# mcahny/vps

Hardware: AMD Instinct MI355X
Metric: frames/sec FuseTrack 1024x2048 (higher is better)
Workload: dtype f32-grade: f16x3 split operands (fp16 pair with scaled residual, 22 significand bits) on MFMA, f32 accumulate

## Files before the change

### include/vps_hip.h

```cpp
#ifndef VPS_HIP_H
#define VPS_HIP_H

#include <stdint.h>

#ifdef __cplusplus
extern "C" {
#endif

int vps_abi_version(void);
const char* vps_build_info(void);

enum { VPS_ACT_NONE = 0, VPS_ACT_RELU = 1, VPS_ACT_LEAKY = 2 };
enum { VPS_PREC_F32 = 0, VPS_PREC_BF16 = 1, VPS_PREC_BF16X3 = 2, VPS_PREC_BF16X6 = 3, VPS_PREC_F16X3 = 4 };

typedef struct vps_conv_desc {
    const float* in;
    int32_t N, H, W;
    int32_t in_ld;
    int32_t in_coff;
    int32_t cin_pad;
    const float* w;
    int32_t cout, cout_pad, kpad;
    int32_t KH, KW, stride;
    int32_t pad_y[2], pad_x[2];
// ... 6 lines not shown
    const float* scale;
    const float* shift;
    const float* res;
    int32_t res_ld, res_coff, res_shift;
    int32_t act;
    float slope;
    const float* offset;
    int32_t off_ld;
    int32_t tile_n;
    int32_t ksplit;
    float* ws;
    int32_t prec;
    const void* w_split;
    int32_t korder;
    int32_t* status;
    double* gn_stats;
    int32_t gn_cpg, gn_rep;
    int32_t* tile_counter;
    const void* w_thin;
} vps_conv_desc;

int vps_conv2d(const vps_conv_desc* d, void* stream);

typedef struct vps_tensor4 {
    float* p;
    int64_t sn, sc, sh, sw;
} vps_tensor4;

int vps_resample2d(vps_tensor4 in, vps_tensor4 flow, vps_tensor4 out,
                   int B, int C, int H, int W, void* stream);

int vps_channelnorm(vps_tensor4 in, vps_tensor4 out, int B, int C, int H, int W, void* stream);

int vps_correlation(const float* in1, int ld1, int coff1, const float* in2, int ld2, int coff2,
                    float* out, int out_ld, int out_coff,
                    int N, int H, int W, int C, int max_disp, int stride2,
                    int act, float slope, void* stream);
int vps_correlation_f16(const float* in1, int ld1, int coff1, const float* in2, int ld2, int coff2,
                        float* out, int out_ld, int out_coff, int N, int H, int W, int C,
                        int max_disp, int stride2, int act, float slope, int32_t* status, void* stream);

int vps_flow_warp(const float* in, int in_ld, int in_coff, const float* flow, int flow_ld, int flow_coff,
                  float* out, int out_ld, int out_coff, int N, int H, int W, int C, void* stream);

int vps_nchw_to_nhwc(const float* in, float* out, int out_ld, int out_coff, int N, int C, int H, int W,
                     int Cpad, void* stream);
// ... 189 lines not shown
```

### vps_amd/csrc/conv_mfma.hip

```cpp
#include "conv_common.h"

namespace {
template <int TM, int TN, int WAVES_M, int WAVES_N, bool DEFORM>
__global__ __launch_bounds__(256, 2)
void conv_mfma_f32_kernel(const vps_conv_desc d, const int M, const int tiles_m, const int tiles_n,
                          const int ksteps_per_split) {
    constexpr int BN = WAVES_N * TN * 32;
    static_assert(WAVES_M * TM * 32 == BM, "block M tile must be 128");
    static_assert(WAVES_M * WAVES_N == 4, "4 wavefronts per block");
    constexpr int NB = BN / 32;

    __shared__ __attribute__((aligned(16))) float As[BM * LDS_LD];
    __shared__ __attribute__((aligned(16))) float Bs[BN * LDS_LD];

    const int t = threadIdx.x;
    int swz = xcd_swizzle(blockIdx.x, gridDim.x);
    int tile_n, tile_m, cls, split;
    decode_tile(d, swz, tiles_n, tiles_m, tile_n, tile_m, cls, split);

    const int py = cls / d.os_x, px = cls - py * d.os_x;
    const int pad_y = d.pad_y[py], pad_x = d.pad_x[px];
    const float* __restrict__ wcls = d.w + (size_t)cls * d.cout_pad * d.kpad;

    const int H = d.H, W = d.W, KH = d.KH, KW = d.KW, cin_pad = d.cin_pad;
// ... 711 lines not shown
        });
        return;
    }
#define VPS_CONV_LAUNCH(KERNEL) hipLaunchKernelGGL((KERNEL), grid, block, 0, s, d, p.M, p.tiles_m, p.tiles_n, p.per_split)
    if (p.kernel == CONV_K_F32) {
        if (d.offset) VPS_CONV_LAUNCH((conv_mfma_f32_kernel<TM, TN, WAVES_M, WAVES_N, true>));
        else VPS_CONV_LAUNCH((conv_mfma_f32_kernel<TM, TN, WAVES_M, WAVES_N, false>));
        return;
    }
    const bool tapmajor = d.korder == 0 && d.KH * d.KW > 1;
    with_prec<true>(d.prec, [&](auto mode) {
        constexpr int MODE = decltype(mode)::value;
        if (d.offset) VPS_CONV_LAUNCH((conv_mfma_bf16p_kernel<TM, TN, WAVES_M, WAVES_N, MODE, false, true>));
        else if (tapmajor) VPS_CONV_LAUNCH((conv_mfma_bf16p_kernel<TM, TN, WAVES_M, WAVES_N, MODE, true>));
        else VPS_CONV_LAUNCH((conv_mfma_bf16p_kernel<TM, TN, WAVES_M, WAVES_N, MODE, false>));
    });
#undef VPS_CONV_LAUNCH
}

conv_switches conv_switches_now(const vps_conv_desc& d) {
    const auto on = [](const char* name) { const char* const e = getenv(name); return !(e && atoi(e) == 0); };
    const auto not0 = [](const char* name) { const char* const e = getenv(name); return !(e && e[0] == '0'); };
    static const bool s2_halo = not0("VPS_S2_HALO"), thin = on("VPS_THIN"), debug_occ = getenv("VPS_DEBUG_OCC") != nullptr;
    conv_switches sw = {true, true, true, true, s2_halo, thin, debug_occ};
    if (d.prec != VPS_PREC_F16X3) return sw;
    if (d.tile_n == 32) {
        if (d.cout > 16) sw.n32 = not0("VPS_N32");
        else if (d.nclass == 4) sw.n16t = on("VPS_N16T");
    } else if (d.tile_n <= 128 && d.KH == 1) sw.pw = on("VPS_PW");
    else if (d.tile_n == 128 && d.KH == 3 && d.stride == 1) sw.h8p = on("VPS_H8P");
    return sw;
}

const conv_limits& conv_limits_once(const bool debug) {
    static const conv_limits lim = [debug] {
        conv_limits l = {};
        int dev = 0;
        (void)hipGetDevice(&dev);
        (void)hipDeviceGetAttribute(&l.cus, hipDeviceAttributeMultiprocessorCount, dev);
        vpsi_conv_pw_limits(l, debug);
        vpsi_conv_thin_limits(l, debug);
        if (debug) vpsi_conv_q_debug_occ();
        return l;
    }();
    return lim;
}

}

extern "C" int vps_conv2d(const vps_conv_desc* dp, void* stream) {
    if (!dp) return VPS_EARG(1);
    const vps_conv_desc& d = *dp;
    if (const int e = vpsi_conv_check(d)) return e;
    const conv_switches sw = conv_switches_now(d);
    const conv_plan p = vpsi_conv_plan(d, conv_limits_once(sw.debug_occ), sw);
    hipStream_t s = (hipStream_t)stream;
    switch (p.kernel) {
        case CONV_K_NONE: return p.err;
        case CONV_K_SMALL3X3V: case CONV_K_SMALL_BATCHED: case CONV_K_SMALL: vpsi_launch_conv_small(d, p, s); break;
        case CONV_K_THIN: vpsi_launch_conv_thin(d, p, s); break;
        case CONV_K_DCN256:
            hipLaunchKernelGGL((conv_mfma_bf16p_kernel<2, 4, 2, 2, VPS_PREC_F16X3, false, true>), dim3(p.grid), dim3(p.block), 0, s, d, p.M, p.tiles_m, p.tiles_n, p.per_split);
            break;
        case CONV_K_N16T: case CONV_K_N32: case CONV_K_N16: vpsi_launch_conv_n16(d, p, s); break;
        case CONV_K_H8S2: vpsi_launch_conv_h8s2(d, p, s); break;
        case CONV_K_H8P: vpsi_launch_conv_h8p(d, p, s); break;
        case CONV_K_H8: vpsi_launch_conv_h8(d, p, s); break;
        case CONV_K_PW: vpsi_launch_conv_pw(d, p, s); break;
        case CONV_K_Q: vpsi_launch_conv_q(d, p, s); break;
        default:
// ... 12 lines not shown
```

### vps_amd/csrc/conv_plan.cpp

```cpp
#include "conv_plan.h"
#include <stdint.h>

namespace {

constexpr int BM = 128, BK = 32;

inline int cdiv(long a, long b) { return (int)((a + b - 1) / b); }
inline size_t in_bytes(const vps_conv_desc& d) { return (size_t)d.N * d.H * d.W * d.in_ld * sizeof(float); }
inline size_t out_bytes(const vps_conv_desc& d) { return (size_t)d.N * d.Ho * d.Wo * d.out_ld * sizeof(float); }
inline bool two_plane(int prec) { return prec == VPS_PREC_F16X3 || prec == VPS_PREC_BF16X3 || prec == VPS_PREC_BF16; }

constexpr int H8_MIN_CHUNKS = 3;
constexpr int PW_MIN_ROUNDS = 2;

conv_plan fail(conv_plan p, int n) { p.kernel = CONV_K_NONE; p.err = VPS_EARG(n); return p; }

conv_plan plan_small(const vps_conv_desc& d, conv_plan p) {
    p.block = 256;
    p.G = 1; p.logG = 0;
    while (p.G < 64 && p.G < (d.cin_pad >> 2)) { p.G <<= 1; ++p.logG; }
    const size_t wbytes = (size_t)(d.cout <= 2 ? 2 : 4) * d.kpad * sizeof(float);
    if (d.KH == 3 && d.KW == 3 && d.stride == 1 && d.nclass == 1 && d.pad_y[0] == 1 && d.pad_x[0] == 1 && d.Ho == d.H && d.Wo == d.W &&
        wbytes <= 150 * 1024 && (d.cout <= 2 || d.cout_pad >= 4) && in_bytes(d) < 0xFFFFFFF0ull &&
        (long)d.N * d.H * d.W < 0x7fffffffL) {
// ... 35 lines not shown
    while (i < 4 && !(d.KH == conv_thin_shapes[i].ks && d.stride == conv_thin_shapes[i].s && d.cin_pad == conv_thin_shapes[i].c4)) ++i;
    if (i == 4) return false;
    const int ph = conv_thin_shapes[i].ph;
    const int tiles_x = (d.Qw + 31) / 32, tiles_y = (d.Qh + ph - 1) / ph;
    const long ntiles = (long)d.N * tiles_x * tiles_y;
    if (ntiles < 512 || ntiles > 0x7fffffffL) return false;
    const int resident = (lim.thin_per_cu[i] > 0 ? lim.thin_per_cu[i] : 1) * (lim.cus > 0 ? lim.cus : 256);
    const long rounds = (ntiles + resident - 1) / resident;
    p.kernel = CONV_K_THIN; p.thin = i; p.tiles_n = tiles_x; p.tiles_m = tiles_y; p.ntiles = (int)ntiles;
    p.grid = (unsigned)((ntiles + rounds - 1) / rounds); p.block = 256;
    return true;
}

bool plan_pw(const vps_conv_desc& d, const conv_limits& lim, const conv_switches& sw, conv_plan& p) {
    if (!sw.pw || d.prec != VPS_PREC_F16X3 || d.offset || d.KH != 1 || d.KW != 1 || d.nclass != 1 || d.ksplit != 1 || d.gn_stats) return false;
    if (d.pad_y[0] || d.pad_x[0] || (d.cin_pad & 31) || d.kpad != d.cin_pad || (d.tile_n != 128 && d.tile_n != 64)) return false;
    const int nk = d.kpad / BK;
    if (nk < 2 || (nk & 1)) return false;
    if (d.Ho != d.Qh || d.Wo != d.Qw || (d.stride == 1 && (d.H != d.Qh || d.W != d.Qw))) return false;
    if (((d.cout | d.out_ld | d.out_coff) & 3) || ((uintptr_t)d.out & 15) || out_bytes(d) >= 0xFFFFFE00ull) return false;
    if (d.res && (((d.res_ld | d.res_coff) & 3) || ((uintptr_t)d.res & 15) || d.res_shift < 0 || d.res_shift > 4 ||
                  (size_t)d.N * (d.Ho >> d.res_shift) * (d.Wo >> d.res_shift) * d.res_ld * sizeof(float) >= 0xFFFFFE00ull)) return false;
    if (in_bytes(d) >= 0xFFFFFE00ull) return false;
    const int per_cu = lim.pw_per_cu[d.tile_n == 128 ? 1 : 0];
    const int resident = (per_cu > 0 ? per_cu : 1) * (lim.cus > 0 ? lim.cus : 256);
    const long total = (long)p.tiles_m * p.tiles_n;
    const int unit = 8 * p.tiles_n;
    if (resident < unit || total < (long)PW_MIN_ROUNDS * resident) return false;
    const long rounds = (total + resident - 1) / resident;
    long grid = (total + rounds - 1) / rounds;
    grid = (grid + unit - 1) / unit * unit;
    if (grid > resident) grid = resident / unit * unit;
    const int mper = (int)(grid / unit);
    p.kernel = CONV_K_PW; p.grid = (unsigned)grid; p.nk = nk; p.nit = (p.tiles_m + mper * 8 - 1) / (mper * 8);
    return true;
}

}

const conv_thin_shape conv_thin_shapes[4] = {{8, 3, 1, 8}, {12, 3, 1, 8}, {4, 7, 2, 8}, {12, 7, 2, 4}};

const char* vpsi_conv_kernel_name(int kernel) {
    static const char* const names[] = {"none", "small3x3v", "small_batched", "small", "thin", "dcn256", "n16t", "n32", "n16",
                                        "h8s2", "h8p", "h8", "halo", "pw", "q", "f32", "bf16p"};
    return kernel >= 0 && kernel <= CONV_K_BF16P ? names[kernel] : "?";
}

int vpsi_conv_check(const vps_conv_desc& d) {
    if (!d.in || !d.out) return VPS_EARG(2);
    if (d.prec < VPS_PREC_F32 || d.prec > VPS_PREC_F16X3) return VPS_EARG(12);
    if (d.prec == VPS_PREC_F32 ? !d.w : !d.w_split) return VPS_EARG(13);
    if ((d.in_ld & 3) || (d.in_coff & 3) || (d.cin_pad & 3) || d.cin_pad <= 0) return VPS_EARG(3);
    if ((d.kpad % BK) || d.kpad < d.KH * d.KW * d.cin_pad || (d.korder != 0 && d.korder != 1)) return VPS_EARG(4);
    if (d.korder == 1 && d.kpad != d.KH * d.KW * ((d.cin_pad + BK - 1) / BK) * BK) return VPS_EARG(14);
    if (d.tile_n != 32 && d.tile_n != 64 && d.tile_n != 128 && !(d.tile_n == 256 && d.offset && d.prec == VPS_PREC_F16X3 && d.korder == 1)) return VPS_EARG(5);
    if (d.cout_pad % d.tile_n || d.cout > d.cout_pad || d.cout <= 0) return VPS_EARG(6);
    if (d.nclass != d.os_y * d.os_x || d.nclass < 1 || d.os_y > 2 || d.os_x > 2) return VPS_EARG(7);
// ... 56 lines not shown
                           d.pad_x[0] >= 0 && d.pad_x[0] <= 1 && d.pad_x[1] >= 0 && d.pad_x[1] <= 1;
        p.tiles_m = (int)tiles2d8; p.block = 512;
        if (fused && d.cout <= 16) { p.kernel = CONV_K_N16T; p.grid = (unsigned)tiles2d8; }
        else { p.kernel = d.cout > 16 ? CONV_K_N32 : CONV_K_N16; p.grid = (unsigned)(tiles2d8 * d.nclass); }
    } else if (h8s2) {
        p.kernel = CONV_K_H8S2; p.tiles_m = (int)tiles2d8; p.block = 512; p.grid = (unsigned)(tiles2d8 * tiles_n * d.ksplit);
    } else if (h8) {
        p.kernel = sw.h8p && d.prec == VPS_PREC_F16X3 && d.KH == 3 ? CONV_K_H8P : CONV_K_H8;
        p.tiles_m = (int)tiles2d8; p.block = 512; p.grid = (unsigned)(tiles2d8 * tiles_n * d.nclass * d.ksplit);
    } else if (halo) {
        const long nblk2 = tiles2d * tiles_n * d.nclass * d.ksplit;
        if (nblk2 > 0x7fffffffL) return fail(p, 21);
        p.kernel = CONV_K_HALO; p.tiles_m = (int)tiles2d; p.grid = (unsigned)nblk2;
    } else {
        p.grid = (unsigned)nblk;
        const bool tapmajor = d.korder == 0 && ntap > 1;
        const bool q_ok = BN >= 64 && !tapmajor;
        if (q_ok && plan_pw(d, lim, sw, p)) return p;
        if (q_ok && !d.offset && two_plane(d.prec)) p.kernel = CONV_K_Q;
        else p.kernel = d.prec == VPS_PREC_F32 ? CONV_K_F32 : CONV_K_BF16P;
    }
    return p;
}
```

### vps_amd/csrc/conv_plan.h

```cpp
#pragma once
#include <stddef.h>
#include "../../include/vps_hip.h"

#ifndef VPS_EARG
#define VPS_EARG(x) (-1000 - (x))
#endif

enum conv_kernel {
    CONV_K_NONE = 0,
    CONV_K_SMALL3X3V,
    CONV_K_SMALL_BATCHED,
    CONV_K_SMALL,
    CONV_K_THIN,
    CONV_K_DCN256,
    CONV_K_N16T,
    CONV_K_N32,
    CONV_K_N16,
    CONV_K_H8S2,
    CONV_K_H8P,
    CONV_K_H8,
    CONV_K_HALO,
    CONV_K_PW,
    CONV_K_Q,
    CONV_K_F32,
    CONV_K_BF16P,
};

struct conv_plan {
    int kernel;
    int err;
    int M;
    int tiles_m, tiles_n;
    int per_split;
    int chunks_per_split;
    unsigned grid, block;
    size_t smem;
    int nk, nit;
    int G, logG, nslot;
    int runs_per_row, total_runs;
    int thin;
    int ntiles;
    bool needs_reduce;
    bool reduce_v4;
};

struct conv_limits {
    int cus;
    int pw_per_cu[2];
    int thin_per_cu[4];
};

struct conv_switches {
    bool pw;
    bool h8p;
    bool n16t;
    bool n32;
    bool s2_halo;
    bool thin;
    bool debug_occ;
};

struct conv_thin_shape { int c4, ks, s, ph; };
extern const conv_thin_shape conv_thin_shapes[4];

int vpsi_conv_check(const vps_conv_desc& d);
conv_plan vpsi_conv_plan(const vps_conv_desc& d, const conv_limits& lim, const conv_switches& sw);
const char* vpsi_conv_kernel_name(int kernel);

#ifdef __HIPCC__
void vpsi_launch_conv_small(const vps_conv_desc& d, const conv_plan& p, hipStream_t s);
void vpsi_launch_conv_thin(const vps_conv_desc& d, const conv_plan& p, hipStream_t s);
void vpsi_launch_conv_n16(const vps_conv_desc& d, const conv_plan& p, hipStream_t s);
void vpsi_launch_conv_h8(const vps_conv_desc& d, const conv_plan& p, hipStream_t s);
void vpsi_launch_conv_h8p(const vps_conv_desc& d, const conv_plan& p, hipStream_t s);
void vpsi_launch_conv_h8s2(const vps_conv_desc& d, const conv_plan& p, hipStream_t s);
void vpsi_launch_conv_pw(const vps_conv_desc& d, const conv_plan& p, hipStream_t s);
void vpsi_launch_conv_q(const vps_conv_desc& d, const conv_plan& p, hipStream_t s);
void vpsi_conv_pw_limits(conv_limits& lim, bool debug);
void vpsi_conv_thin_limits(conv_limits& lim, bool debug);
void vpsi_conv_q_debug_occ();
#endif
```

### vps_amd/csrc/conv_pw.hip

```cpp
#include "conv_common.h"
#include <cstdio>

namespace {

constexpr int PMODE = VPS_PREC_F16X3;

template <int TN, bool HAS_RES, int NKU>
__global__ __launch_bounds__(256, 2)
void conv_pw_kernel(const vps_conv_desc d, const int M, const int tiles_m, const int tiles_n, const int nk, const int nit) {
    constexpr int TM = 2, WAVES_N = 2;
    constexpr int BN = WAVES_N * TN * 32;
    typedef Split<PMODE> SM;
    typedef _Float16 elem_t;
    typedef vec8<elem_t> x8;
    typedef vec4<elem_t> x4;
    constexpr int NSA = SM::NSA, NSB = SM::NSB, NLB = SM::NLB, NT = SM::NT;
    static_assert(NSA == 2 && NLB == 2 && NSB == 3 && NT == 3, "f16x3");
    constexpr int ABUF = NSA * BM * LDS_LDH;
    constexpr int NFRAG = NLB * 2 * (BN / 32);
    constexpr int BBUF = NFRAG * 512;
    static_assert((NFRAG * 64) % 256 == 0, "whole 16-byte chunks per thread");
    constexpr int NBL = NFRAG * 64 / 256;
    constexpr int NST = TM * TN * 4;

    __shared__ __attribute__((aligned(16))) elem_t As[2 * ABUF];
    __shared__ __attribute__((aligned(16))) elem_t Bs[2 * BBUF];
    __shared__ __attribute__((aligned(16))) float scsh[2 * BN];

    const int t = threadIdx.x;
    const int lane = t & 63;
    const int wave = __builtin_amdgcn_readfirstlane(t >> 6);
    const int wm = wave / WAVES_N, wn = wave - wm * WAVES_N;

    const int G = gridDim.x;
    const int xcd = blockIdx.x & 7, bj = blockIdx.x >> 3;
    const int tile_n = bj % tiles_n, mlocal = bj / tiles_n, mper = (G >> 3) / tiles_n;

    const int k4 = t & 7;
    const int r0 = t >> 3;
    const int nbt = d.cout_pad >> 5, kst = d.kpad >> 4;
    const size_t wplane = (size_t)nbt * kst * 512;
    const __amdgpu_buffer_rsrc_t wrsrc = make_rsrc(d.w_split, (unsigned)(wplane * NSB * sizeof(elem_t)));
    const unsigned wbase = (unsigned)((((size_t)(tile_n * (BN / 32)) * kst) * 512) * sizeof(elem_t));
    const unsigned wlane = (unsigned)lane * 16u;
    const __amdgpu_buffer_rsrc_t arsrc = make_rsrc(d.in, (unsigned)((size_t)d.N * d.H * d.W * d.in_ld * sizeof(float)));
    const __amdgpu_buffer_rsrc_t orsrc = make_rsrc(d.out, (unsigned)((size_t)d.N * d.Ho * d.Wo * d.out_ld * sizeof(float)));
    const int rs = d.res_shift;
    const __amdgpu_buffer_rsrc_t rrsrc = make_rsrc(HAS_RES ? d.res : d.in, HAS_RES ? (unsigned)((size_t)d.N * (d.Ho >> rs) * (d.Wo >> rs) * d.res_ld * sizeof(float)) : 0u);
    const unsigned ld4 = (unsigned)d.in_ld * 4u;
    const unsigned acoff = (unsigned)(d.in_coff + k4 * 4) * 4u;
    const bool plain = d.stride == 1;

    int lk = 0, lit = 0, bk = 0;
    unsigned rowoff[4];
    auto set_rows = [&](const int it) {
        const int tm = (it * mper + mlocal) * 8 + xcd;
#pragma unroll
        for (int i = 0; i < 4; ++i) {
            const int m = tm * BM + r0 + 32 * i;
            const bool ok = tm < tiles_m && m < M;
            unsigned pix = (unsigned)m;
            if (!plain) {
                const int mm = ok ? m : 0;
                const int qx = mm % d.Qw, tq = mm / d.Qw;
                const int qy = tq % d.Qh, n = tq / d.Qh;
                pix = (unsigned)((n * d.H + qy * d.stride) * d.W + qx * d.stride);
            }
            rowoff[i] = ok ? pix * ld4 + acoff : 0xFFFFFFF0u;
        }
    };
    f32x4 areg[2][4];
    x8 breg[2][NBL];
    float amax = 0.f;

    auto load_A = [&](const int slot) {
        const unsigned koff = (unsigned)lk * (BK * 4u);
#pragma unroll
        for (int i = 0; i < 4; ++i)
            areg[slot][i] = buffer_load16<f32x4>(arsrc, rowoff[i] != 0xFFFFFFF0u ? rowoff[i] + koff : 0xFFFFFFF0u, 0u);
        if (++lk == nk) {
            lk = 0;
            ++lit;
            set_rows(lit);
        }
    };
    auto load_B = [&](const int slot) {
#pragma unroll
        for (int j = 0; j < NBL; ++j) {
            const int f = wave + 4 * j, bcol = f % (BN / 32), pm = f / (BN / 32);
            breg[slot][j] = buffer_load16<x8>(wrsrc, wlane, wbase + (unsigned)(((size_t)(pm >> 1) * wplane + ((size_t)bcol * kst + 2 * bk + (pm & 1)) * 512) * sizeof(elem_t)));
        }
        if (++bk == nk) bk = 0;
    };
    auto store_A = [&](const int i, const int buf, const int slot) {
        x4 sp[NSA];
        split_act<PMODE>(areg[slot][i], sp, amax);
        const int row = r0 + 32 * i;
#pragma unroll
        for (int p = 0; p < NSA; ++p)
            *reinterpret_cast<x4*>(&As[buf * ABUF + p * (BM * LDS_LDH) + row * LDS_LDH + (((k4 >> 1) ^ lds_swz(row)) << 3) + ((k4 & 1) << 2)]) = sp[p];
    };
    auto store_B = [&](const int j, const int buf, const int slot) {
        *reinterpret_cast<x8*>(&Bs[buf * BBUF + (t + 256 * j) * 8]) = breg[slot][j];
    };

    const int frag_row = (wm * TM * 32 + (lane & 31)) * LDS_LDH;
    const int frag_sw = lds_swz(lane & 31);
    const int frag_chunk[2] = {(((lane >> 5)) ^ frag_sw) << 3, ((2 + (lane >> 5)) ^ frag_sw) << 3};
    x8 af[2][NSA][TM];
    x8 bf[NSB][TN];
    auto read_A = [&](const int m, const int buf) {
#pragma unroll
        for (int p = 0; p < NSA; ++p)
#pragma unroll
            for (int a = 0; a < TM; ++a)
                af[m][p][a] = *reinterpret_cast<const x8*>(&As[buf * ABUF + p * (BM * LDS_LDH) + a * 32 * LDS_LDH + frag_row + frag_chunk[m]]);
    };
    auto read_B = [&](const int m, const int p, const int buf) {
#pragma unroll
        for (int b = 0; b < TN; ++b)
            bf[p][b] = *reinterpret_cast<const x8*>(&Bs[buf * BBUF + (((p * 2 + m) * (BN / 32)) + wn * TN + b) * 512 + lane * 8]);
    };

    f32x16 acc[TM][TN];

    {
        const int c = t & (BN - 1);
        const int co = tile_n * BN + c;
        float v = t < BN ? 1.f : 0.f;
        if (co < d.cout) {
            if (t < BN && d.scale) v = d.scale[co];
            if (t >= BN && d.shift) v = d.shift[co];
        }
        if (t < 2 * BN) scsh[t] = v;
    }
    set_rows(0);
    load_B(0);
    load_A(0);
#pragma unroll
    for (int i = 0; i < 4; ++i) store_A(i, 0, 0);
#pragma unroll
    for (int j = 0; j < NBL; ++j) store_B(j, 0, 0);
    load_B(1);
    load_A(1);
    if constexpr (NKU == 2) {
#pragma unroll
        for (int j = 0; j < NBL; ++j) store_B(j, 1, 1);
    } else {
        load_B(0);
    }
    load_A(0);
    {
        const u32x4 z = {0u, 0u, 0u, 0u};
#pragma unroll
        for (int i = 0; i < NST; ++i) __builtin_amdgcn_raw_buffer_store_b128(z, orsrc, (int)(0xFFFFFE00u + 16u * (unsigned)i), 0, 0);
    }
    __syncthreads();

    constexpr int NM1 = NT * TM * TN;
    constexpr int NW = 8;

    auto kstep = [&](auto cur_tag, auto first_tag) {
        constexpr int cur = decltype(cur_tag)::value;
        constexpr bool first = decltype(first_tag)::value;
        constexpr int slot = cur ^ 1;
        read_A(0, cur);
#pragma unroll
        for (int p = 0; p < NLB; ++p) read_B(0, p, cur);
        read_A(1, cur);
        __builtin_amdgcn_sched_barrier(0);
        auto prep = [&](const int q) {
            if (SM::PB[q] >= NLB) {
#pragma unroll
                for (int b = 0; b < TN; ++b) bf[SM::PB[q]][b] = derive_weight_plane<PMODE>(bf[0][b]);
            }
        };
#pragma unroll
        for (int q = 0; q < NT; ++q) {
            prep(q);
#pragma unroll
            for (int a = 0; a < TM; ++a)
#pragma unroll
                for (int b = 0; b < TN; ++b) {
                    if (first && q == 0) {
                        const f32x16 z = {0.f, 0.f, 0.f, 0.f, 0.f, 0.f, 0.f, 0.f, 0.f, 0.f, 0.f, 0.f, 0.f, 0.f, 0.f, 0.f};
                        acc[a][b] = split_mfma<PMODE>(bf[SM::PB[q]][b], af[0][SM::PA[q]][a], z);
                    } else {
                        acc[a][b] = split_mfma<PMODE>(bf[SM::PB[q]][b], af[0][SM::PA[q]][a], acc[a][b]);
                    }
                }
            bool last_use = SM::PB[q] < NLB;
#pragma unroll
            for (int q2 = q + 1; q2 < NT; ++q2) last_use = last_use && SM::PB[q2] != SM::PB[q];
#pragma unroll
            for (int q2 = q + 1; q2 < NT; ++q2) last_use = last_use && !(SM::PB[q] == 0 && SM::PB[q2] >= NLB);
            if (last_use) {
                __builtin_amdgcn_sched_barrier(0);
                read_B(1, SM::PB[q], cur);
                __builtin_amdgcn_sched_barrier(0);
            }
        }
        auto work = [&](const int w) {
            if (w < 4) store_A(w, cur ^ 1, slot);
            else if (w == 4) {
                if constexpr (NKU != 2) {
#pragma unroll
                    for (int j = 0; j < (NBL + 1) / 2; ++j) store_B(j, cur ^ 1, slot);
                }
            } else if (w == 5) {
                if constexpr (NKU != 2) {
#pragma unroll
                    for (int j = (NBL + 1) / 2; j < NBL; ++j) store_B(j, cur ^ 1, slot);
                }
            } else if (w == 6) {
                if constexpr (NKU != 2) load_B(slot);
            } else load_A(slot);
        };
        int mf = 0;
#pragma unroll
        for (int q = 0; q < NT; ++q) {
            prep(q);
#pragma unroll
            for (int a = 0; a < TM; ++a)
#pragma unroll
                for (int b = 0; b < TN; ++b) {
                    acc[a][b] = split_mfma<PMODE>(bf[SM::PB[q]][b], af[1][SM::PA[q]][a], acc[a][b]);
                    ++mf;
#pragma unroll
                    for (int w = 0; w < NW; ++w) {
                        const int pos = ((w + 1) * NM1 + NW) / (NW + 1);
                        if (mf == (pos < 1 ? 1 : (pos > NM1 ? NM1 : pos))) {
                            __builtin_amdgcn_sched_barrier(0);
                            work(w);
                            __builtin_amdgcn_sched_barrier(0);
                        }
                    }
                }
        }
        __syncthreads();
    };

    const int prow = lane & 31;
    const int cl = wn * TN * 32 + 4 * (lane >> 5);
    const unsigned ocol4 = (unsigned)(d.out_coff + tile_n * BN + cl) * 4u;
    const unsigned rcol4 = (unsigned)(d.res_coff + tile_n * BN + cl) * 4u;
    const float ns = d.act == VPS_ACT_RELU ? 0.f : (d.act == VPS_ACT_LEAKY ? d.slope : 1.f);
    auto epilogue = [&](const int it) {
        const int tm = (it * mper + mlocal) * 8 + xcd;
        unsigned ooff[TM], roff[TM];
#pragma unroll
        for (int a = 0; a < TM; ++a) {
            const int m = tm * BM + wm * TM * 32 + a * 32 + prow;
            const bool inside = tm < tiles_m && m < M;
            ooff[a] = inside ? (unsigned)m * ((unsigned)d.out_ld * 4u) + ocol4 : 0xFFFFFFF0u;
            roff[a] = 0xFFFFFFF0u;
            if constexpr (HAS_RES) {
                unsigned rp = (unsigned)m;
                if (rs) {
                    const int mm = inside ? m : 0;
                    const int qx = mm % d.Qw, tq = mm / d.Qw;
                    const int qy = tq % d.Qh, n = tq / d.Qh;
                    rp = (unsigned)((n * (d.Ho >> rs) + (qy >> rs)) * (d.Wo >> rs) + (qx >> rs));
                }
                roff[a] = inside ? rp * ((unsigned)d.res_ld * 4u) + rcol4 : 0xFFFFFFF0u;
            }
        }
        f32x4 rv[HAS_RES ? TM : 1][HAS_RES ? TN : 1][4];
        if constexpr (HAS_RES) {
#pragma unroll
            for (int a = 0; a < TM; ++a)
#pragma unroll
                for (int b = 0; b < TN; ++b)
#pragma unroll
                    for (int g = 0; g < 4; ++g) {
                        const bool cok = tile_n * BN + cl + b * 32 + 8 * g < d.cout;
// ... 50 lines not shown
            kstep(C0{}, FF{});
            kstep(C1{}, FF{});
            ks += 2;
            if (ks == nk) {
                epilogue(it);
                ++it;
                ks = 0;
#pragma unroll
                for (int a = 0; a < TM; ++a)
#pragma unroll
                    for (int b = 0; b < TN; ++b)
#pragma unroll
                        for (int r = 0; r < 16; ++r) acc[a][b][r] = 0.f;
            }
        }
    }
    report_range<PMODE>(d, amax);
}

}

__attribute__((visibility("hidden")))
void vpsi_conv_pw_limits(conv_limits& lim, bool debug) {
    (void)hipOccupancyMaxActiveBlocksPerMultiprocessor(&lim.pw_per_cu[0], conv_pw_kernel<1, false, 0>, 256, 0);
    (void)hipOccupancyMaxActiveBlocksPerMultiprocessor(&lim.pw_per_cu[1], conv_pw_kernel<2, false, 0>, 256, 0);
    if (debug) for (int tn = 1; tn <= 2; ++tn) fprintf(stderr, "[vps] pointwise kernel <TN %d>: %d blocks/CU\n", tn, lim.pw_per_cu[tn - 1]);
}

__attribute__((visibility("hidden")))
void vpsi_launch_conv_pw(const vps_conv_desc& d, const conv_plan& p, hipStream_t s) {
    const int tn = d.tile_n == 128 ? 2 : 1;
#define VPS_PW_LAUNCH(TNV, RESV, NKV) hipLaunchKernelGGL((conv_pw_kernel<TNV, RESV, NKV>), dim3(p.grid), dim3(p.block), 0, s, d, p.M, p.tiles_m, p.tiles_n, p.nk, p.nit)
#define VPS_PW_NK(TNV, RESV)                                         \
    do {                                                             \
        if (p.nk == 2) VPS_PW_LAUNCH(TNV, RESV, 2);                  \
        else if (p.nk == 4) VPS_PW_LAUNCH(TNV, RESV, 4);             \
        else if (p.nk == 8) VPS_PW_LAUNCH(TNV, RESV, 8);             \
        else VPS_PW_LAUNCH(TNV, RESV, 0);                            \
    } while (0)
    if (d.res) { if (tn == 2) VPS_PW_NK(2, true); else VPS_PW_NK(1, true); }
    else { if (tn == 2) VPS_PW_NK(2, false); else VPS_PW_NK(1, false); }
#undef VPS_PW_NK
#undef VPS_PW_LAUNCH
}
```

### vps_amd/hip.py

```python
import ctypes
import os
from ctypes import (POINTER, Structure, byref, c_char_p, c_double, c_float, c_int, c_int32, c_int64, c_uint64,
                    c_void_p)

import torch

_HERE = os.path.dirname(os.path.abspath(__file__))
LIB_PATH = os.environ.get('VPS_HIP_LIB') or os.path.join(_HERE, 'csrc', 'libvpship.so')
ABI_VERSION = 21

ACT_NONE, ACT_RELU, ACT_LEAKY = 0, 1, 2
PREC_F32, PREC_BF16, PREC_BF16X3, PREC_BF16X6, PREC_F16X3 = 0, 1, 2, 3, 4

SYMBOLS = [
    'vps_abi_version', 'vps_build_info', 'vps_conv2d', 'vps_resample2d', 'vps_channelnorm', 'vps_correlation',
    'vps_flow_warp', 'vps_nchw_to_nhwc', 'vps_nhwc_to_nchw', 'vps_resize', 'vps_pool3x3s2', 'vps_bfp_gather',
    'vps_bfp_scatter', 'vps_bfp_scatter_all', 'vps_axpb', 'vps_flow_prep', 'vps_flow_prep_pad', 'vps_flow_stage', 'vps_flow_stage_full', 'vps_groupnorm_relu', 'vps_groupnorm_apply', 'vps_tcea_temporal',
    'vps_tcea_modulate', 'vps_tcea_modulate_ld', 'vps_correlation_f16', 'vps_roi_align', 'vps_nms_batched', 'vps_delta2bbox', 'vps_bbox_overlaps',
    'vps_row_softmax', 'vps_mask_count', 'vps_mask_commit', 'vps_mask_removal', 'vps_mask_removal_dep', 'vps_mask_removal_hist', 'vps_frame_tail', 'vps_mask_level', 'vps_panoptic_combine',
    'vps_panoptic_combine_dev', 'vps_rpn_select', 'vps_rpn_collect', 'vps_maskroi_select', 'vps_maskroi_finish', 'vps_track_assign', 'vps_pan_instances',
    'vps_unify_hist', 'vps_unify_tables', 'vps_unify_write', 'vps_image_prep', 'vps_resize_u8', 'vps_segment_stats', 'vps_segment_paint', 'vps_pair_count',
    'vps_png_info', 'vps_png_decode_bgr8', 'vps_jpeg_info', 'vps_jpeg_decode_coef', 'vps_jpeg_reconstruct',
    'vps_png_encode_bound', 'vps_png_deflate',
    'vps_png_inflate', 'vps_png_reconstruct_ws', 'vps_png_reconstruct', 'vps_png_reconstruct_block_rows',
    'vps_unify_tables_image', 'vps_segment_stats_ch', 'vps_segment_paint_ch', 'vps_sseg_confusion',
    'vps_overlay_render', 'vps_jpeg_quant_tables', 'vps_jpeg_encode_bound', 'vps_jpeg_encode_coef', 'vps_jpeg_write_bound', 'vps_jpeg_write',
    'vps_flow_max_radius', 'vps_flow_colour',
    'vps_rle_runs', 'vps_rle_runs_ws', 'vps_rle_band_rows', 'vps_rle_strings', 'vps_rle_strings_bound',
]


class ConvDesc(Structure):
    _fields_ = [
        ('inp', c_void_p), ('N', c_int32), ('H', c_int32), ('W', c_int32),
        ('in_ld', c_int32), ('in_coff', c_int32), ('cin_pad', c_int32),
        ('w', c_void_p), ('cout', c_int32), ('cout_pad', c_int32), ('kpad', c_int32),
        ('KH', c_int32), ('KW', c_int32), ('stride', c_int32),
        ('pad_y', c_int32 * 2), ('pad_x', c_int32 * 2),
# ... 46 lines not shown
def load_host():
    load()
    return _host


def load():
    global _lib
    if _lib is not None:
        return _lib
    if not os.path.exists(LIB_PATH):
        raise VpsHipError('libvpship.so not found at %s — build it with `python -c "import __graft_entry__ as g; '
                          'g.build()"` or `make -C vps_amd/csrc`. There is no CPU fallback.' % LIB_PATH)
    lib = ctypes.PyDLL(LIB_PATH)
    missing = [s for s in SYMBOLS if not hasattr(lib, s)]
    if missing:
        raise VpsHipError('libvpship.so is missing symbols: %s' % missing)
    lib.vps_abi_version.restype = c_int
    lib.vps_build_info.restype = c_char_p
    if lib.vps_abi_version() != ABI_VERSION:
        raise VpsHipError('libvpship.so ABI %d != binding ABI %d' % (lib.vps_abi_version(), ABI_VERSION))
    for s in SYMBOLS[2:]:
        getattr(lib, s).restype = c_int
    lib.vps_conv2d.argtypes = [POINTER(ConvDesc), c_void_p]
    lib.vps_resample2d.argtypes = [Tensor4, Tensor4, Tensor4, c_int, c_int, c_int, c_int, c_void_p]
    lib.vps_channelnorm.argtypes = [Tensor4, Tensor4, c_int, c_int, c_int, c_int, c_void_p]
    lib.vps_correlation.argtypes = [c_void_p, c_int, c_int, c_void_p, c_int, c_int, c_void_p, c_int, c_int,
                                    c_int, c_int, c_int, c_int, c_int, c_int, c_int, c_float, c_void_p]
    lib.vps_correlation_f16.argtypes = [c_void_p, c_int, c_int, c_void_p, c_int, c_int, c_void_p, c_int, c_int,
                                        c_int, c_int, c_int, c_int, c_int, c_int, c_int, c_float, c_void_p, c_void_p]
    lib.vps_flow_warp.argtypes = [c_void_p, c_int, c_int, c_void_p, c_int, c_int, c_void_p, c_int, c_int,
                                  c_int, c_int, c_int, c_int, c_void_p]
    lib.vps_nchw_to_nhwc.argtypes = [c_void_p, c_void_p, c_int, c_int, c_int, c_int, c_int, c_int, c_int, c_void_p]
    lib.vps_nhwc_to_nchw.argtypes = [c_void_p, c_int, c_int, c_void_p, c_int, c_int, c_int, c_int, c_void_p]
    lib.vps_resize.argtypes = [c_void_p, c_int, c_int, c_int, c_int, c_void_p, c_int, c_int, c_int, c_int,
                               c_int, c_int, c_int, c_float, c_void_p]
    lib.vps_pool3x3s2.argtypes = [c_void_p, c_int, c_int, c_int, c_int, c_void_p, c_int, c_int, c_int, c_int, c_int,
                                  c_void_p]
    lib.vps_bfp_gather.argtypes = [POINTER(c_void_p), POINTER(c_int), POINTER(c_int), c_int, c_void_p, c_int, c_int,
                                   c_int, c_int, c_int, c_int, c_void_p]
    lib.vps_bfp_scatter.argtypes = [c_void_p, c_int, c_void_p, c_int, c_void_p, c_int, c_int, c_int, c_int, c_int,
                                    c_int, c_void_p]
    lib.vps_bfp_scatter_all.argtypes = [c_void_p, c_int, POINTER(c_void_p), POINTER(c_int), POINTER(c_void_p), POINTER(c_int), c_int, c_int, c_int,
                                        c_int, c_int, c_void_p]
    lib.vps_axpb.argtypes = [c_void_p, c_int, c_int, c_void_p, c_int, c_int, c_int64, c_int, c_float, c_float,
                             c_void_p]
    lib.vps_flow_prep.argtypes = [c_void_p, c_void_p, c_void_p, c_void_p, c_void_p, c_int, c_int, c_int, c_void_p,
# ... 114 lines not shown
def check(code, what):
    if code != 0:
        raise VpsHipError('%s failed with code %d (negative hipError_t, or -1000-x = bad argument x)' % (what, code))


def ptr(t):
    if t is None:
        return None
    if not t.is_cuda:
        raise VpsHipError('libvpship kernels need device tensors (got a CPU tensor); there is no CPU path')
    return c_void_p(t.data_ptr())


def tensor4_nchw(t):
    assert t.dim() == 4 and t.dtype == torch.float32
    if not t.is_cuda:
        raise VpsHipError('libvpship kernels need device tensors')
    s = t.stride()
    return Tensor4(c_void_p(t.data_ptr()), s[0], s[1], s[2], s[3])


def conv2d(desc):
    check(load().vps_conv2d(byref(desc), stream_ptr()), 'vps_conv2d')
```

### vps_amd/nhwc.py

```python
import collections
import ctypes
import os
import weakref
from ctypes import c_float, c_int, c_void_p

import torch

from . import hip


def _ceil(a, b):
    return (a + b - 1) // b * b


_PREC_NAMES = {'f32': hip.PREC_F32, 'bf16': hip.PREC_BF16, 'bf16x3': hip.PREC_BF16X3, 'bf16x6': hip.PREC_BF16X6, 'f16x3': hip.PREC_F16X3}
PREC_NAMES = _PREC_NAMES
_PLANES = {hip.PREC_BF16: 1, hip.PREC_BF16X3: 2, hip.PREC_BF16X6: 3, hip.PREC_F16X3: 3}
MFMA_PRODUCTS = {hip.PREC_F32: 1, hip.PREC_BF16: 1, hip.PREC_BF16X3: 3, hip.PREC_BF16X6: 6, hip.PREC_F16X3: 3}
F16_SLOTS = 4096
_F16_STATUS = {}
_F16_LAYERS = {}
_F16_NEXT = [1]
F16_FALLBACKS = [0]

# ... 401 lines not shown

    def __call__(self, x, out=None, ws=None, name=None, res=None, res_shift=0, offset=None, act=None, gn=None, temp=False, keep=False):
        if self._mfma_twin is not None and x.N * x.H * x.W >= 100000:
            return self._mfma_twin(x, out, ws, name, res, res_shift, offset, act, gn, temp, keep)
        assert x.C == self.cin or (x.C >= self.cin and x.C <= self.cin_pad), (x.C, self.cin)
        assert x.coff % 4 == 0 and x.ld % 4 == 0 and x.coff + self.cin_pad <= x.ld, (x.coff, x.ld, self.cin_pad)
        Ho, Wo = self.out_hw(x.H, x.W)
        if out is None:
            out = ws.fmap(name, x.N, Ho, Wo, self.cout, temp=temp, out=keep)
        assert (out.N, out.H, out.W) == (x.N, Ho, Wo) and out.C == self.cout, ((out.N, out.H, out.W, out.C), (x.N, Ho, Wo, self.cout))
        key = (x.t.data_ptr(), x.N, x.H, x.W, x.ld, x.coff, out.t.data_ptr(), out.ld, out.coff,
               None if res is None else (res.t.data_ptr(), res.ld, res.coff, res_shift),
               None if offset is None else (offset.t.data_ptr(), offset.ld), act, _stream_key(),
               None if gn is None else (gn[0].data_ptr(), gn[1]))
        hit = self._launches.get(key)
        if hit is not None and CONV_TRACE is None:
            d = hit.desc
            self.gn_fused = bool(d.gn_stats)
            hip.conv2d(d)
            return out
        Qh, Qw = (x.H, x.W) if self.transposed else (Ho, Wo)
        geo = conv_geometry(self, x.N, Qh, Qw, out.ld, out.coff, res is not None, None if gn is None else gn[1])
        d = self._describe(x, out, Qh, Qw, res, res_shift, offset, act, gn, geo)
        scratch = self._scratch(d, geo, ws, x.t.device)
        self.gn_fused = geo.gn_cpg > 0
        self._launch(d, x, res is not None)
        if len(self._launches) >= 16:
            self._launches.clear()
        self._launches[key] = _Launch(d, (scratch, x.t, out.t, None if res is None else res.t, None if offset is None else offset.t))
        return out

    def _describe(self, x, out, Qh, Qw, res, res_shift, offset, act, gn, geo):
        d = hip.ConvDesc()
        d.inp = x.t.data_ptr(); d.N, d.H, d.W = x.N, x.H, x.W
        d.in_ld, d.in_coff, d.cin_pad = x.ld, x.coff, self.cin_pad
        d.prec, d.korder = self.prec, self.korder
        if self.prec == hip.PREC_F32:
            d.w = self.w.data_ptr()
        else:
            d.w_split = self.w_split.data_ptr()
            if self.w_thin is not None:
                d.w_thin = self.w_thin.data_ptr()
        if self.prec == hip.PREC_F16X3:
            d.status = f16_status(x.t.device).data_ptr() + 4 * self.f16_slot
        d.cout, d.cout_pad, d.kpad = self.cout, self.cout_pad, self.kpad
        d.KH, d.KW, d.stride = self.KH, self.KW, self.stride
# ... 196 lines not shown
```

Before: 55.95.

## Add 64-row pointwise conv tile variant and prefer it over K-split

```diff
diff --git a/include/vps_hip.h b/include/vps_hip.h
--- a/include/vps_hip.h
+++ b/include/vps_hip.h
@@ -52,6 +52,8 @@
 
 int vps_conv2d(const vps_conv_desc* d, void* stream);
 
+int vps_conv_pw_unsplit(const vps_conv_desc* d);
+
 typedef struct vps_tensor4 {
     float* p;
     int64_t sn, sc, sh, sw;
diff --git a/vps_amd/csrc/conv_mfma.hip b/vps_amd/csrc/conv_mfma.hip
--- a/vps_amd/csrc/conv_mfma.hip
+++ b/vps_amd/csrc/conv_mfma.hip
@@ -757,12 +757,16 @@
     const auto on = [](const char* name) { const char* const e = getenv(name); return !(e && atoi(e) == 0); };
     const auto not0 = [](const char* name) { const char* const e = getenv(name); return !(e && e[0] == '0'); };
     static const bool s2_halo = not0("VPS_S2_HALO"), thin = on("VPS_THIN"), debug_occ = getenv("VPS_DEBUG_OCC") != nullptr;
-    conv_switches sw = {true, true, true, true, s2_halo, thin, debug_occ};
+    conv_switches sw = {true, true, true, true, s2_halo, thin, debug_occ, true, false};
     if (d.prec != VPS_PREC_F16X3) return sw;
     if (d.tile_n == 32) {
         if (d.cout > 16) sw.n32 = not0("VPS_N32");
         else if (d.nclass == 4) sw.n16t = on("VPS_N16T");
-    } else if (d.tile_n <= 128 && d.KH == 1) sw.pw = on("VPS_PW");
+    } else if (d.tile_n <= 128 && d.KH == 1) {
+        sw.pw = on("VPS_PW");
+        const char* const e = getenv("VPS_PW_SMALL");
+        sw.pw_small = !(e && atoi(e) == 0); sw.pw_small_any = e && atoi(e) == 2;
+    }
     else if (d.tile_n == 128 && d.KH == 3 && d.stride == 1) sw.h8p = on("VPS_H8P");
     return sw;
 }
@@ -773,6 +777,7 @@
         int dev = 0;
         (void)hipGetDevice(&dev);
         (void)hipDeviceGetAttribute(&l.cus, hipDeviceAttributeMultiprocessorCount, dev);
+        l.xcds = l.cus >= 64 && l.cus % 8 == 0 ? 8 : 1;
         vpsi_conv_pw_limits(l, debug);
         vpsi_conv_thin_limits(l, debug);
         if (debug) vpsi_conv_q_debug_occ();
@@ -781,6 +786,12 @@
     return lim;
 }
 
+}
+
+extern "C" int vps_conv_pw_unsplit(const vps_conv_desc* dp) {
+    if (!dp) return 0;
+    const conv_switches sw = conv_switches_now(*dp);
+    return vpsi_conv_pw_unsplit(*dp, conv_limits_once(sw.debug_occ), sw) ? 1 : 0;
 }
 
 extern "C" int vps_conv2d(const vps_conv_desc* dp, void* stream) {
diff --git a/vps_amd/csrc/conv_plan.cpp b/vps_amd/csrc/conv_plan.cpp
--- a/vps_amd/csrc/conv_plan.cpp
+++ b/vps_amd/csrc/conv_plan.cpp
@@ -81,17 +81,27 @@
     if (d.res && (((d.res_ld | d.res_coff) & 3) || ((uintptr_t)d.res & 15) || d.res_shift < 0 || d.res_shift > 4 ||
                   (size_t)d.N * (d.Ho >> d.res_shift) * (d.Wo >> d.res_shift) * d.res_ld * sizeof(float) >= 0xFFFFFE00ull)) return false;
     if (in_bytes(d) >= 0xFFFFFE00ull) return false;
-    const int per_cu = lim.pw_per_cu[d.tile_n == 128 ? 1 : 0];
-    const int resident = (per_cu > 0 ? per_cu : 1) * (lim.cus > 0 ? lim.cus : 256);
-    const long total = (long)p.tiles_m * p.tiles_n;
-    const int unit = 8 * p.tiles_n;
-    if (resident < unit || total < (long)PW_MIN_ROUNDS * resident) return false;
+    const int cus = lim.cus > 0 ? lim.cus : 256, xcds = lim.xcds > 0 ? lim.xcds : 8;
+    const int unit = xcds * p.tiles_n;
+    const int tn = d.tile_n == 128 ? 1 : 0;
+    int rows = BM, tiles_m = p.tiles_m;
+    int resident = (lim.pw_per_cu[tn] > 0 ? lim.pw_per_cu[tn] : 1) * cus;
+    long total = (long)tiles_m * p.tiles_n;
+    if (resident < unit || total < (long)PW_MIN_ROUNDS * resident || sw.pw_small_any) {
+        if (!sw.pw_small || lim.pw64_per_cu[tn] <= 0) return false;
+        if (total >= 2L * cus && nk > 8 && !sw.pw_small_any) return false;
+        rows = BM / 2; tiles_m = cdiv(p.M, rows);
+        resident = lim.pw64_per_cu[tn] * cus;
+        total = (long)tiles_m * p.tiles_n;
+        if (resident < unit || (total < cus && !sw.pw_small_any)) return false;
+    }
     const long rounds = (total + resident - 1) / resident;
     long grid = (total + rounds - 1) / rounds;
     grid = (grid + unit - 1) / unit * unit;
     if (grid > resident) grid = resident / unit * unit;
     const int mper = (int)(grid / unit);
-    p.kernel = CONV_K_PW; p.grid = (unsigned)grid; p.nk = nk; p.nit = (p.tiles_m + mper * 8 - 1) / (mper * 8);
+    p.kernel = CONV_K_PW; p.grid = (unsigned)grid; p.nk = nk; p.nit = (tiles_m + mper * xcds - 1) / (mper * xcds);
+    p.tiles_m = tiles_m; p.pw_rows = rows; p.xcds = xcds;
     return true;
 }
 
@@ -194,3 +204,11 @@
     }
     return p;
 }
+
+bool vpsi_conv_pw_unsplit(const vps_conv_desc& d, const conv_limits& lim, const conv_switches& sw) {
+    vps_conv_desc u = d;
+    u.ksplit = 1; u.ws = nullptr; u.tile_counter = nullptr;
+    if (vpsi_conv_check(u)) return false;
+    const conv_plan p = vpsi_conv_plan(u, lim, sw);
+    return p.kernel == CONV_K_PW && p.pw_rows == BM / 2;
+}
diff --git a/vps_amd/csrc/conv_plan.h b/vps_amd/csrc/conv_plan.h
--- a/vps_amd/csrc/conv_plan.h
+++ b/vps_amd/csrc/conv_plan.h
@@ -36,6 +36,7 @@
     unsigned grid, block;
     size_t smem;
     int nk, nit;
+    int pw_rows, xcds;
     int G, logG, nslot;
     int runs_per_row, total_runs;
     int thin;
@@ -48,6 +49,8 @@
     int cus;
     int pw_per_cu[2];
     int thin_per_cu[4];
+    int pw64_per_cu[2];
+    int xcds;
 };
 
 struct conv_switches {
@@ -58,6 +61,8 @@
     bool s2_halo;
     bool thin;
     bool debug_occ;
+    bool pw_small;
+    bool pw_small_any;
 };
 
 struct conv_thin_shape { int c4, ks, s, ph; };
@@ -66,6 +71,7 @@
 int vpsi_conv_check(const vps_conv_desc& d);
 conv_plan vpsi_conv_plan(const vps_conv_desc& d, const conv_limits& lim, const conv_switches& sw);
 const char* vpsi_conv_kernel_name(int kernel);
+bool vpsi_conv_pw_unsplit(const vps_conv_desc& d, const conv_limits& lim, const conv_switches& sw);
 
 #ifdef __HIPCC__
 void vpsi_launch_conv_small(const vps_conv_desc& d, const conv_plan& p, hipStream_t s);
diff --git a/vps_amd/csrc/conv_pw.hip b/vps_amd/csrc/conv_pw.hip
--- a/vps_amd/csrc/conv_pw.hip
+++ b/vps_amd/csrc/conv_pw.hip
@@ -5,10 +5,12 @@
 
 constexpr int PMODE = VPS_PREC_F16X3;
 
-template <int TN, bool HAS_RES, int NKU>
+template <int TM, int TN, bool HAS_RES, int NKU>
 __global__ __launch_bounds__(256, 2)
-void conv_pw_kernel(const vps_conv_desc d, const int M, const int tiles_m, const int tiles_n, const int nk, const int nit) {
-    constexpr int TM = 2, WAVES_N = 2;
+void conv_pw_kernel(const vps_conv_desc d, const int M, const int tiles_m, const int tiles_n, const int nk, const int nit, const int nx) {
+    constexpr int WAVES_N = 2;
+    constexpr int BMT = 2 * TM * 32;
+    constexpr int NA = BMT / 32;
     constexpr int BN = WAVES_N * TN * 32;
     typedef Split<PMODE> SM;
     typedef _Float16 elem_t;
@@ -16,7 +18,7 @@
     typedef vec4<elem_t> x4;
     constexpr int NSA = SM::NSA, NSB = SM::NSB, NLB = SM::NLB, NT = SM::NT;
     static_assert(NSA == 2 && NLB == 2 && NSB == 3 && NT == 3, "f16x3");
-    constexpr int ABUF = NSA * BM * LDS_LDH;
+    constexpr int ABUF = NSA * BMT * LDS_LDH;
     constexpr int NFRAG = NLB * 2 * (BN / 32);
     constexpr int BBUF = NFRAG * 512;
     static_assert((NFRAG * 64) % 256 == 0, "whole 16-byte chunks per thread");
@@ -33,8 +35,8 @@
     const int wm = wave / WAVES_N, wn = wave - wm * WAVES_N;
 
     const int G = gridDim.x;
-    const int xcd = blockIdx.x & 7, bj = blockIdx.x >> 3;
-    const int tile_n = bj % tiles_n, mlocal = bj / tiles_n, mper = (G >> 3) / tiles_n;
+    const int bj = blockIdx.x / nx, xcd = blockIdx.x - bj * nx;
+    const int tile_n = bj % tiles_n, mlocal = bj / tiles_n, mper = (G / nx) / tiles_n;
 
     const int k4 = t & 7;
     const int r0 = t >> 3;
@@ -52,12 +54,12 @@
     const bool plain = d.stride == 1;
 
     int lk = 0, lit = 0, bk = 0;
-    unsigned rowoff[4];
+    unsigned rowoff[NA];
     auto set_rows = [&](const int it) {
-        const int tm = (it * mper + mlocal) * 8 + xcd;
-#pragma unroll
-        for (int i = 0; i < 4; ++i) {
-            const int m = tm * BM + r0 + 32 * i;
+        const int tm = (it * mper + mlocal) * nx + xcd;
+#pragma unroll
+        for (int i = 0; i < NA; ++i) {
+            const int m = tm * BMT + r0 + 32 * i;
             const bool ok = tm < tiles_m && m < M;
             unsigned pix = (unsigned)m;
             if (!plain) {
@@ -69,14 +71,14 @@
             rowoff[i] = ok ? pix * ld4 + acoff : 0xFFFFFFF0u;
         }
     };
-    f32x4 areg[2][4];
+    f32x4 areg[2][NA];
     x8 breg[2][NBL];
     float amax = 0.f;
 
     auto load_A = [&](const int slot) {
         const unsigned koff = (unsigned)lk * (BK * 4u);
 #pragma unroll
-        for (int i = 0; i < 4; ++i)
+        for (int i = 0; i < NA; ++i)
             areg[slot][i] = buffer_load16<f32x4>(arsrc, rowoff[i] != 0xFFFFFFF0u ? rowoff[i] + koff : 0xFFFFFFF0u, 0u);
         if (++lk == nk) {
             lk = 0;
@@ -98,7 +100,7 @@
         const int row = r0 + 32 * i;
 #pragma unroll
         for (int p = 0; p < NSA; ++p)
-            *reinterpret_cast<x4*>(&As[buf * ABUF + p * (BM * LDS_LDH) + row * LDS_LDH + (((k4 >> 1) ^ lds_swz(row)) << 3) + ((k4 & 1) << 2)]) = sp[p];
+            *reinterpret_cast<x4*>(&As[buf * ABUF + p * (BMT * LDS_LDH) + row * LDS_LDH + (((k4 >> 1) ^ lds_swz(row)) << 3) + ((k4 & 1) << 2)]) = sp[p];
     };
     auto store_B = [&](const int j, const int buf, const int slot) {
         *reinterpret_cast<x8*>(&Bs[buf * BBUF + (t + 256 * j) * 8]) = breg[slot][j];
@@ -114,7 +116,7 @@
         for (int p = 0; p < NSA; ++p)
 #pragma unroll
             for (int a = 0; a < TM; ++a)
-                af[m][p][a] = *reinterpret_cast<const x8*>(&As[buf * ABUF + p * (BM * LDS_LDH) + a * 32 * LDS_LDH + frag_row + frag_chunk[m]]);
+                af[m][p][a] = *reinterpret_cast<const x8*>(&As[buf * ABUF + p * (BMT * LDS_LDH) + a * 32 * LDS_LDH + frag_row + frag_chunk[m]]);
     };
     auto read_B = [&](const int m, const int p, const int buf) {
 #pragma unroll
@@ -138,7 +140,7 @@
     load_B(0);
     load_A(0);
 #pragma unroll
-    for (int i = 0; i < 4; ++i) store_A(i, 0, 0);
+    for (int i = 0; i < NA; ++i) store_A(i, 0, 0);
 #pragma unroll
     for (int j = 0; j < NBL; ++j) store_B(j, 0, 0);
     load_B(1);
@@ -158,7 +160,7 @@
     __syncthreads();
 
     constexpr int NM1 = NT * TM * TN;
-    constexpr int NW = 8;
+    constexpr int NW = NA + 4;
 
     auto kstep = [&](auto cur_tag, auto first_tag) {
         constexpr int cur = decltype(cur_tag)::value;
@@ -201,18 +203,18 @@
             }
         }
         auto work = [&](const int w) {
-            if (w < 4) store_A(w, cur ^ 1, slot);
-            else if (w == 4) {
+            if (w < NA) store_A(w, cur ^ 1, slot);
+            else if (w == NA) {
                 if constexpr (NKU != 2) {
 #pragma unroll
                     for (int j = 0; j < (NBL + 1) / 2; ++j) store_B(j, cur ^ 1, slot);
                 }
-            } else if (w == 5) {
+            } else if (w == NA + 1) {
                 if constexpr (NKU != 2) {
 #pragma unroll
                     for (int j = (NBL + 1) / 2; j < NBL; ++j) store_B(j, cur ^ 1, slot);
                 }
-            } else if (w == 6) {
+            } else if (w == NA + 2) {
                 if constexpr (NKU != 2) load_B(slot);
             } else load_A(slot);
         };
@@ -246,11 +248,11 @@
     const unsigned rcol4 = (unsigned)(d.res_coff + tile_n * BN + cl) * 4u;
     const float ns = d.act == VPS_ACT_RELU ? 0.f : (d.act == VPS_ACT_LEAKY ? d.slope : 1.f);
     auto epilogue = [&](const int it) {
-        const int tm = (it * mper + mlocal) * 8 + xcd;
+        const int tm = (it * mper + mlocal) * nx + xcd;
         unsigned ooff[TM], roff[TM];
 #pragma unroll
         for (int a = 0; a < TM; ++a) {
-            const int m = tm * BM + wm * TM * 32 + a * 32 + prow;
+            const int m = tm * BMT + wm * TM * 32 + a * 32 + prow;
             const bool inside = tm < tiles_m && m < M;
             ooff[a] = inside ? (unsigned)m * ((unsigned)d.out_ld * 4u) + ocol4 : 0xFFFFFFF0u;
             roff[a] = 0xFFFFFFF0u;
@@ -347,24 +349,33 @@
 
 __attribute__((visibility("hidden")))
 void vpsi_conv_pw_limits(conv_limits& lim, bool debug) {
-    (void)hipOccupancyMaxActiveBlocksPerMultiprocessor(&lim.pw_per_cu[0], conv_pw_kernel<1, false, 0>, 256, 0);
-    (void)hipOccupancyMaxActiveBlocksPerMultiprocessor(&lim.pw_per_cu[1], conv_pw_kernel<2, false, 0>, 256, 0);
-    if (debug) for (int tn = 1; tn <= 2; ++tn) fprintf(stderr, "[vps] pointwise kernel <TN %d>: %d blocks/CU\n", tn, lim.pw_per_cu[tn - 1]);
+    (void)hipOccupancyMaxActiveBlocksPerMultiprocessor(&lim.pw_per_cu[0], conv_pw_kernel<2, 1, false, 0>, 256, 0);
+    (void)hipOccupancyMaxActiveBlocksPerMultiprocessor(&lim.pw_per_cu[1], conv_pw_kernel<2, 2, false, 0>, 256, 0);
+    (void)hipOccupancyMaxActiveBlocksPerMultiprocessor(&lim.pw64_per_cu[0], conv_pw_kernel<1, 1, false, 0>, 256, 0);
+    (void)hipOccupancyMaxActiveBlocksPerMultiprocessor(&lim.pw64_per_cu[1], conv_pw_kernel<1, 2, false, 0>, 256, 0);
+    if (debug) for (int tn = 1; tn <= 2; ++tn)
+        fprintf(stderr, "[vps] pointwise kernel <TN %d>: %d blocks/CU on 128-row tiles, %d on 64-row tiles\n", tn, lim.pw_per_cu[tn - 1], lim.pw64_per_cu[tn - 1]);
 }
 
 __attribute__((visibility("hidden")))
 void vpsi_launch_conv_pw(const vps_conv_desc& d, const conv_plan& p, hipStream_t s) {
     const int tn = d.tile_n == 128 ? 2 : 1;
-#define VPS_PW_LAUNCH(TNV, RESV, NKV) hipLaunchKernelGGL((conv_pw_kernel<TNV, RESV, NKV>), dim3(p.grid), dim3(p.block), 0, s, d, p.M, p.tiles_m, p.tiles_n, p.nk, p.nit)
-#define VPS_PW_NK(TNV, RESV)                                         \
+#define VPS_PW_LAUNCH(TMV, TNV, RESV, NKV) hipLaunchKernelGGL((conv_pw_kernel<TMV, TNV, RESV, NKV>), dim3(p.grid), dim3(p.block), 0, s, d, p.M, p.tiles_m, p.tiles_n, p.nk, p.nit, p.xcds)
+#define VPS_PW_NK(TMV, TNV, RESV)                                    \
     do {                                                             \
-        if (p.nk == 2) VPS_PW_LAUNCH(TNV, RESV, 2);                  \
-        else if (p.nk == 4) VPS_PW_LAUNCH(TNV, RESV, 4);             \
-        else if (p.nk == 8) VPS_PW_LAUNCH(TNV, RESV, 8);             \
-        else VPS_PW_LAUNCH(TNV, RESV, 0);                            \
+        if (p.nk == 2) VPS_PW_LAUNCH(TMV, TNV, RESV, 2);             \
+        else if (p.nk == 4) VPS_PW_LAUNCH(TMV, TNV, RESV, 4);        \
+        else if (p.nk == 8) VPS_PW_LAUNCH(TMV, TNV, RESV, 8);        \
+        else VPS_PW_LAUNCH(TMV, TNV, RESV, 0);                       \
     } while (0)
-    if (d.res) { if (tn == 2) VPS_PW_NK(2, true); else VPS_PW_NK(1, true); }
-    else { if (tn == 2) VPS_PW_NK(2, false); else VPS_PW_NK(1, false); }
+#define VPS_PW_TM(TNV, RESV)                                         \
+    do {                                                             \
+        if (p.pw_rows == 64) VPS_PW_NK(1, TNV, RESV);                \
+        else VPS_PW_NK(2, TNV, RESV);                                \
+    } while (0)
+    if (d.res) { if (tn == 2) VPS_PW_TM(2, true); else VPS_PW_TM(1, true); }
+    else { if (tn == 2) VPS_PW_TM(2, false); else VPS_PW_TM(1, false); }
+#undef VPS_PW_TM
 #undef VPS_PW_NK
 #undef VPS_PW_LAUNCH
 }
diff --git a/vps_amd/hip.py b/vps_amd/hip.py
--- a/vps_amd/hip.py
+++ b/vps_amd/hip.py
@@ -13,7 +13,7 @@
 PREC_F32, PREC_BF16, PREC_BF16X3, PREC_BF16X6, PREC_F16X3 = 0, 1, 2, 3, 4
 
 SYMBOLS = [
-    'vps_abi_version', 'vps_build_info', 'vps_conv2d', 'vps_resample2d', 'vps_channelnorm', 'vps_correlation',
+    'vps_abi_version', 'vps_build_info', 'vps_conv2d', 'vps_conv_pw_unsplit', 'vps_resample2d', 'vps_channelnorm', 'vps_correlation',
     'vps_flow_warp', 'vps_nchw_to_nhwc', 'vps_nhwc_to_nchw', 'vps_resize', 'vps_pool3x3s2', 'vps_bfp_gather',
     'vps_bfp_scatter', 'vps_bfp_scatter_all', 'vps_axpb', 'vps_flow_prep', 'vps_flow_prep_pad', 'vps_flow_stage', 'vps_flow_stage_full', 'vps_groupnorm_relu', 'vps_groupnorm_apply', 'vps_tcea_temporal',
     'vps_tcea_modulate', 'vps_tcea_modulate_ld', 'vps_correlation_f16', 'vps_roi_align', 'vps_nms_batched', 'vps_delta2bbox', 'vps_bbox_overlaps',
@@ -106,6 +106,7 @@
     for s in SYMBOLS[2:]:
         getattr(lib, s).restype = c_int
     lib.vps_conv2d.argtypes = [POINTER(ConvDesc), c_void_p]
+    lib.vps_conv_pw_unsplit.argtypes = [POINTER(ConvDesc)]
     lib.vps_resample2d.argtypes = [Tensor4, Tensor4, Tensor4, c_int, c_int, c_int, c_int, c_void_p]
     lib.vps_channelnorm.argtypes = [Tensor4, Tensor4, c_int, c_int, c_int, c_int, c_void_p]
     lib.vps_correlation.argtypes = [c_void_p, c_int, c_int, c_void_p, c_int, c_int, c_void_p, c_int, c_int,
@@ -266,3 +267,7 @@
 
 def conv2d(desc):
     check(load().vps_conv2d(byref(desc), stream_ptr()), 'vps_conv2d')
+
+
+def conv_pw_unsplit(desc):
+    return load().vps_conv_pw_unsplit(byref(desc)) == 1
diff --git a/vps_amd/nhwc.py b/vps_amd/nhwc.py
--- a/vps_amd/nhwc.py
+++ b/vps_amd/nhwc.py
@@ -447,6 +447,9 @@
         Qh, Qw = (x.H, x.W) if self.transposed else (Ho, Wo)
         geo = conv_geometry(self, x.N, Qh, Qw, out.ld, out.coff, res is not None, None if gn is None else gn[1])
         d = self._describe(x, out, Qh, Qw, res, res_shift, offset, act, gn, geo)
+        if geo.ksplit > 1 and self.KH == 1 and self.KW == 1 and self.prec == hip.PREC_F16X3 and hip.conv_pw_unsplit(d):
+            geo = ConvGeometry(geo.tile_n, 1, geo.gn_cpg, 0, 0)
+            d.ksplit = 1
         scratch = self._scratch(d, geo, ws, x.t.device)
         self.gn_fused = geo.gn_cpg > 0
         self._launch(d, x, res is not None)
```

After: 55.72. No clear change (-0.4%).
